# CogitoNTNU/geoguessr-ai

Hardware: AMD Instinct MI355X
Metric: images/sec TinyViT-21M-224 train, 4-heading batch (higher is better)
Workload: dtype fp32 (bf16x3 split MFMA); 1 GPU; tiny_vit_21m_224 4x224x224 panoramas, fwd+bwd+AdamW, soft-CE over 12647 geocells, freeze_all_but_last_stage, DropPath, train-mode BN; panoramas_per_gpu=256, images_per_gpu=1024, global_batch_panoramas=256, parallelism=dp1, precision=fp32_split

## Files before the change

### geoguessr-ai_amd/csrc/attention.hip

```cpp
#include "common.h"
#include <stdlib.h>
#include "../../include/gg.h"
int gg_attention_flash_bwd_impl(const GgAttnArgs* a, int dtype, int forward_rounded_bias, void* stream);

struct AttnParams {
    const bf16* qkv; int64_t ld;
    int q_off, k_off, v_off, head_stride;
    bf16* out; int64_t ldo;
    const bf16* bias; int nbias;
    int ws, nWx, nWy, H, W;
    int ws_inv;
    int N;
    int nh;
    float scale;
    const bf16* dout; int64_t lddo;
    bf16* dqkv;
    float* dbias;
    float* dbias_part;
    float* lse;
};

__device__ __forceinline__ int attn_origin(const AttnParams& p, int w) {
    if (p.ws == 0) return w * p.N;
    const int per_img = p.nWx * p.nWy;
// ... 614 lines not shown
    __shared__ __attribute__((aligned(16))) float row_lse[2][Np], row_delta[2][Np];
    __shared__ float dbias_s[DBIAS ? DBC * 256 : 1];
    __shared__ __attribute__((aligned(4))) unsigned char ci[Np], cj[Np];
    const int bid = gg_xcd_remap(blockIdx.x, gridDim.x);
    const int wb = bid / p.nh, h = bid % p.nh;
    const int lane = threadIdx.x & 63, wave = threadIdx.x >> 6;
    const int lr = lane & 15, lg = lane >> 4;
    const int qcol = p.q_off + h * p.head_stride, kcol = p.k_off + h * p.head_stride, vcol = p.v_off + h * p.head_stride;
    const int ocol = h * D;
    const int nt = (p.N + 15) / 16;
    const int ti = wave * 16 + lr;
    for (int t = threadIdx.x; t < Np; t += blockDim.x) {
        const int tt = min(t, p.N - 1), i = (tt * p.ws_inv) >> 16;
        ci[t] = p.ws ? (unsigned char)i : 0;
        cj[t] = p.ws ? (unsigned char)(tt - i * p.ws) : 0;
    }
    if (DBIAS) { for (int t = threadIdx.x; t < DBC * 256; t += blockDim.x) dbias_s[t] = 0.f; }
    u32x2 bq[NKT], bk[NKT];
#pragma unroll
    for (int kt = 0; kt < NKT; ++kt) {
        const int c0 = kt * 16 + lg * 4;
        bq[kt] = p.bias ? *reinterpret_cast<const u32x2*>(p.bias + ((int64_t)h * Np + ti) * Np + c0) : attn_mask_raw(c0, p.N);
        bk[kt] = p.bias ? *reinterpret_cast<const u32x2*>(p.bias + ((int64_t)h * Np + min(ti, p.N - 1)) * Np + c0) : attn_mask_raw(c0, p.N);
    }
    const float c2 = p.scale * 1.4426950408889634f;
    const int w0 = wb * GW, w1 = min(num_windows, w0 + GW);
    bf16x8 qr[IT], kr[IT], vr[IT], dr[IT], orr[IT];
    float lse_r = 0.f;
    auto fetch = [&](int w) {
        const int origin = attn_origin(p, w);
        int tokv[IT];
        attn_stage_tokens<D, Np>(p, origin, tokv);
        attn_load_rows<D, Np>(qr, p.qkv, p.ld, qcol, tokv);
        attn_load_rows<D, Np>(kr, p.qkv, p.ld, kcol, tokv);
        attn_load_rows<D, Np>(vr, p.qkv, p.ld, vcol, tokv);
        attn_load_rows<D, Np>(dr, p.dout, p.lddo, ocol, tokv);
        attn_load_rows<D, Np>(orr, p.out, p.ldo, ocol, tokv);
        if (threadIdx.x < Np) {
            const int tk = attn_token(p, origin, threadIdx.x);
            lse_r = tk >= 0 ? -1.4426950408889634f * p.lse[(int64_t)tk * p.nh + h] : 0.f;
        }
    };
    f32x4 dsum[DBIAS ? NKT : 1];
#pragma unroll
    for (int kt = 0; kt < (DBIAS ? NKT : 1); ++kt) dsum[kt] = (f32x4){0.f, 0.f, 0.f, 0.f};
    if (w0 < w1) fetch(w0);
    for (int w = w0; w < w1; ++w) {
        const int sel = (w - w0) & 1;
        bf16* Qs = img[sel][0]; bf16* Ks = img[sel][1]; bf16* Vs = img[sel][2]; bf16* dOs = img[sel][3];
        attn_store_rows<D, Np>(Qs, RS, qr);
        attn_store_rows<D, Np>(Ks, RS, kr);
        attn_store_rows<D, Np>(Vs, RS, vr);
        attn_store_rows<D, Np>(dOs, RS, dr);
        if (threadIdx.x < Np) row_lse[sel][threadIdx.x] = lse_r;
#pragma unroll
        for (int i = 0; i < IT; ++i) {
            const int idx = threadIdx.x + i * 256;
            float sm = 0.f;
#pragma unroll
            for (int j = 0; j < 8; ++j) sm += (float)dr[i][j] * (float)orr[i][j];
#pragma unroll
            for (int o = 1; o < CH; o <<= 1) sm += __shfl_xor(sm, o, 64);
            if (idx < Np * CH && (idx % CH) == 0) row_delta[sel][idx / CH] = -sm;
        }
        const int origin = attn_origin(p, w);
        const int tok_own = wave < nt ? attn_token(p, origin, ti) : -1;
        __syncthreads();
        if (w + 1 < w1) fetch(w + 1);
        if (wave < nt) {
            {
                bf16x8 qf[KS], dof[KS];
#pragma unroll
                for (int ks = 0; ks < KS; ++ks) {
                    qf[ks] = attn_lds_row_frag(Qs, RS, ti, ks * 32 + lg * 8);
                    dof[ks] = attn_lds_row_frag(dOs, RS, ti, ks * 32 + lg * 8);
                }
                const float nlse_q = row_lse[sel][ti], ndelta_q = row_delta[sel][ti];
                f32x4 dq[DT];
#pragma unroll
                for (int dt = 0; dt < DT; ++dt) dq[dt] = (f32x4){0.f, 0.f, 0.f, 0.f};
#pragma unroll
                for (int kp = 0; kp < NKT / 2; ++kp) {
                    f32x4 dst[2];
#pragma unroll
                    for (int u = 0; u < 2; ++u) {
                        const int kt = kp * 2 + u;
                        f32x4 acc = attn_bias_cvt(bq[kt]), acc2 = {ndelta_q, ndelta_q, ndelta_q, ndelta_q};
#pragma unroll
                        for (int ks = 0; ks < KS; ++ks) {
                            const bf16x8 kf = attn_lds_row_frag(Ks, RS, kt * 16 + lr, ks * 32 + lg * 8);
                            const bf16x8 vf = attn_lds_row_frag(Vs, RS, kt * 16 + lr, ks * 32 + lg * 8);
                            acc = __builtin_amdgcn_mfma_f32_16x16x32_bf16(kf, qf[ks], acc, 0, 0, 0);
                            acc2 = __builtin_amdgcn_mfma_f32_16x16x32_bf16(vf, dof[ks], acc2, 0, 0, 0);
                        }
                        const int key0 = kt * 16 + lg * 4;
#pragma unroll
                        for (int r = 0; r < 4; ++r) acc2[r] *= __builtin_amdgcn_exp2f(fmaf(acc[r], c2, nlse_q));
                        if (DBIAS) dsum[kt] += acc2;
                        dst[u] = acc2;
                    }
                    const bf16x8 df = attn_pack(dst[0], dst[1]);
#pragma unroll
                    for (int dt = 0; dt < DT; ++dt) {
                        const bf16x8 kf = attn_lds_tr_frag(Ks, RS, dt * 16, kp * 32, lr, lg);
                        dq[dt] = __builtin_amdgcn_mfma_f32_16x16x32_bf16(kf, df, dq[dt], 0, 0, 0);
                    }
                }
                if (tok_own >= 0) {
#pragma unroll
                    for (int dt = 0; dt < DT; ++dt) {
                        bf16x4 ov = {(bf16)(dq[dt][0] * p.scale), (bf16)(dq[dt][1] * p.scale), (bf16)(dq[dt][2] * p.scale), (bf16)(dq[dt][3] * p.scale)};
                        *reinterpret_cast<bf16x4*>(p.dqkv + (int64_t)tok_own * p.ld + qcol + dt * 16 + lg * 4) = ov;
                    }
                }
            }
            {
                bf16x8 kf[KS], vf[KS];
#pragma unroll
                for (int ks = 0; ks < KS; ++ks) {
                    kf[ks] = attn_lds_row_frag(Ks, RS, ti, ks * 32 + lg * 8);
                    vf[ks] = attn_lds_row_frag(Vs, RS, ti, ks * 32 + lg * 8);
                }
                f32x4 dk[DT], dv[DT];
#pragma unroll
                for (int dt = 0; dt < DT; ++dt) { dk[dt] = (f32x4){0.f, 0.f, 0.f, 0.f}; dv[dt] = (f32x4){0.f, 0.f, 0.f, 0.f}; }
#pragma unroll
                for (int qp = 0; qp < NKT / 2; ++qp) {
                    f32x4 pt[2], dst[2];
#pragma unroll
                    for (int u = 0; u < 2; ++u) {
                        const int qt = qp * 2 + u;
                        const int q0 = qt * 16 + lg * 4;
                        const f32x4 l4 = *reinterpret_cast<const f32x4*>(&row_lse[sel][q0]);
                        f32x4 acc = attn_bias_cvt(bk[qt]), acc2 = *reinterpret_cast<const f32x4*>(&row_delta[sel][q0]);
#pragma unroll
                        for (int ks = 0; ks < KS; ++ks) {
                            const bf16x8 qf = attn_lds_row_frag(Qs, RS, qt * 16 + lr, ks * 32 + lg * 8);
                            const bf16x8 dof = attn_lds_row_frag(dOs, RS, qt * 16 + lr, ks * 32 + lg * 8);
                            acc = __builtin_amdgcn_mfma_f32_16x16x32_bf16(qf, kf[ks], acc, 0, 0, 0);
                            acc2 = __builtin_amdgcn_mfma_f32_16x16x32_bf16(dof, vf[ks], acc2, 0, 0, 0);
                        }
#pragma unroll
                        for (int r = 0; r < 4; ++r) {
                            const float pr = __builtin_amdgcn_exp2f(fmaf(acc[r], c2, l4[r]));
                            acc[r] = pr;
                            acc2[r] *= pr;
                        }
                        pt[u] = acc;
                        dst[u] = acc2;
                    }
                    const bf16x8 pf = attn_pack(pt[0], pt[1]);
                    const bf16x8 df = attn_pack(dst[0], dst[1]);
#pragma unroll
                    for (int dt = 0; dt < DT; ++dt) {
                        const bf16x8 qtf = attn_lds_tr_frag(Qs, RS, dt * 16, qp * 32, lr, lg);
                        const bf16x8 dotf = attn_lds_tr_frag(dOs, RS, dt * 16, qp * 32, lr, lg);
                        dk[dt] = __builtin_amdgcn_mfma_f32_16x16x32_bf16(qtf, df, dk[dt], 0, 0, 0);
                        dv[dt] = __builtin_amdgcn_mfma_f32_16x16x32_bf16(dotf, pf, dv[dt], 0, 0, 0);
                    }
                }
                if (tok_own >= 0) {
#pragma unroll
                    for (int dt = 0; dt < DT; ++dt) {
                        bf16x4 a = {(bf16)(dk[dt][0] * p.scale), (bf16)(dk[dt][1] * p.scale), (bf16)(dk[dt][2] * p.scale), (bf16)(dk[dt][3] * p.scale)};
                        bf16x4 b = {(bf16)dv[dt][0], (bf16)dv[dt][1], (bf16)dv[dt][2], (bf16)dv[dt][3]};
                        *reinterpret_cast<bf16x4*>(p.dqkv + (int64_t)tok_own * p.ld + kcol + dt * 16 + lg * 4) = a;
                        *reinterpret_cast<bf16x4*>(p.dqkv + (int64_t)tok_own * p.ld + vcol + dt * 16 + lg * 4) = b;
                    }
                }
            }
        }
    }
    if (DBIAS) {
        if (wave < nt && ti < p.N) {
            const int qci = ci[ti], qcj = cj[ti];
#pragma unroll
            for (int kt = 0; kt < NKT; ++kt) {
                const int key0 = kt * 16 + lg * 4;
#pragma unroll
                for (int r = 0; r < 4; ++r)
                    if (key0 + r < p.N) atomicAdd(&dbias_s[(lr & (DBC - 1)) * 256 + abs(qci - (int)ci[key0 + r]) * p.ws + abs(qcj - (int)cj[key0 + r])], dsum[kt][r]);
            }
        }
        __syncthreads();
        for (int t = threadIdx.x; t < p.nbias; t += blockDim.x) {
            float sum = 0.f;
#pragma unroll
            for (int c = 0; c < DBC; ++c) sum += dbias_s[c * 256 + t];
            if (p.dbias_part) p.dbias_part[((int64_t)wb * p.nh + h) * p.nbias + t] = sum;
            else atomicAdd(&p.dbias[h * p.nbias + t], sum);
        }
    }
}

__global__ void attn_dbias_final_kernel(const float* __restrict__ rows, int nrows, int W, float* __restrict__ dbias) {
    const int i = blockIdx.x * blockDim.x + threadIdx.x;
    if (i >= W) return;
    double s = 0.0;
    for (int r = 0; r < nrows; ++r) s += (double)rows[(int64_t)r * W + i];
    dbias[i] += (float)s;
}

static int attn_fill(AttnParams& p, const GgAttnArgs* a, const char* who) {
    GG_CHECK(a && a->qkv, "%s: null qkv", who);
    GG_CHECK(a->head_dim == 32 || a->head_dim == 64, "%s: head_dim must be 32 or 64 (got %d)", who, a->head_dim);
    GG_CHECK(a->tokens_per_window > 0 && a->tokens_per_window <= 256,
             "%s: %d tokens per window unsupported (max 256: full-row softmax in registers)", who, a->tokens_per_window);
    GG_CHECK(a->num_windows > 0 && a->num_heads > 0, "%s: bad window/head count", who);
    GG_CHECK((a->ld & 7) == 0 && (a->q_off & 7) == 0 && (a->k_off & 7) == 0 && (a->v_off & 7) == 0 && (a->head_stride & 7) == 0,
             "%s: qkv offsets/strides must be multiples of 8 elements", who);
    if (a->window_size > 0) {
        GG_CHECK(a->window_size * a->window_size == a->tokens_per_window, "%s: window_size^2 != tokens_per_window", who);
        GG_CHECK(a->map_h % a->window_size == 0 && a->map_w % a->window_size == 0, "%s: map not divisible by window", who);
        GG_CHECK(a->num_windows % ((a->map_h / a->window_size) * (a->map_w / a->window_size)) == 0, "%s: window count", who);
        GG_CHECK(a->window_size <= 16, "%s: window_size > 16 unsupported", who);
    }
    if (a->bias || a->dbias) GG_CHECK(a->window_size > 0 && a->tokens_per_window <= 256, "%s: bias needs a window geometry", who);
    if (a->bias) GG_CHECK(((uintptr_t)a->bias & 7) == 0, "%s: expanded bias must be 8-byte aligned", who);
    p.qkv = (const bf16*)a->qkv; p.ld = a->ld;
    p.q_off = a->q_off; p.k_off = a->k_off; p.v_off = a->v_off; p.head_stride = a->head_stride;
    p.out = (bf16*)a->out; p.ldo = a->ldo;
    p.bias = (const bf16*)a->bias; p.nbias = a->window_size * a->window_size;
    p.ws = a->window_size;
    p.ws_inv = a->window_size ? (65536 + a->window_size - 1) / a->window_size : 0;
    p.H = a->map_h; p.W = a->map_w;
    p.nWx = a->window_size ? a->map_w / a->window_size : 1;
    p.nWy = a->window_size ? a->map_h / a->window_size : 1;
    p.N = a->tokens_per_window; p.nh = a->num_heads; p.scale = a->scale;
    p.dout = (const bf16*)a->dout; p.lddo = a->lddo; p.dqkv = (bf16*)a->dqkv; p.dbias = a->dbias; p.dbias_part = a->dbias ? a->dbias_scratch : nullptr; p.lse = a->lse;
    return 0;
}
static int attn_nkt(int N) { return N <= 64 ? 4 : (N <= 160 ? 10 : (N <= 224 ? 14 : 16)); }
extern "C" int gg_attention_padded_tokens(int tokens_per_window) { return 16 * attn_nkt(tokens_per_window); }
extern "C" int gg_attention_expand_bias(const float* table, int num_heads, int window_size, float scale, void* full, void* stream) {
    GG_CHECK(table && full && num_heads > 0 && window_size > 0 && window_size <= 16 && scale > 0.f, "gg_attention_expand_bias: bad args");
    const int N = window_size * window_size, Np = 16 * attn_nkt(N);
    const int64_t total = (int64_t)num_heads * Np * Np;
    hipLaunchKernelGGL(attn_expand_bias_kernel, dim3((unsigned)std::min<int64_t>(gg_cdiv(total, 256), 4096)), dim3(256), 0, (hipStream_t)stream,
                       table, num_heads, window_size, N, Np, 1.0f / scale, (bf16*)full);
    GG_LAUNCH_CHECK();
    return 0;
}

static bool attn_use_flash(const GgAttnArgs* a) { return a && (a->tokens_per_window > 256 || a->window_size > 16); }
static bool attn_use_split_bwd(const GgAttnArgs* a) {
    static const bool nosplit = gg_dev_env("GG_ATTN_NO_SPLIT") != nullptr;
    if (!a || nosplit || a->head_dim != 32 || a->window_size <= 0) return false;
    const int nt16 = (a->tokens_per_window + 15) / 16;
    return (nt16 == 13 || nt16 == 9) && (!a->bias || a->bias_table);
}
extern "C" int gg_attention_fwd(const GgAttnArgs* a, void* stream) {
    if (attn_use_flash(a)) {
        GG_CHECK(!a->bias || a->bias_table, "gg_attention_fwd: this window shape takes the bias as bias_table (compact f32)");
        return gg_attention_flash_fwd(a, 0, stream);
    }
    AttnParams p;
    GG_TRY(attn_fill(p, a, "gg_attention_fwd"));
    GG_CHECK(a->out && (a->ldo & 3) == 0, "gg_attention_fwd: bad out");
    dim3 grid((unsigned)(a->num_windows * a->num_heads)), block(256);
    hipStream_t s = (hipStream_t)stream;
    GG_PROF(GG_CAT_ATTN, 4.0 * a->num_windows * a->num_heads * (double)p.N * p.N * a->head_dim, 8.0 * a->num_windows * a->num_heads * (double)p.N * a->head_dim, stream);
    const int nkt = attn_nkt(p.N);
#define GG_FWD(D_, K_) hipLaunchKernelGGL((attn_fwd_kernel<D_, K_>), grid, block, 0, s, p)
    static const char* small_env = gg_dev_env("GG_ATTN_SMALL");
    if (a->head_dim == 32 && nkt == 4 && !(small_env && small_env[0] == '0') && a->num_windows >= 64) {
        constexpr int GW = 8;
        const dim3 g2((unsigned)(gg_cdiv(a->num_windows, GW) * a->num_heads));
        hipLaunchKernelGGL((attn_fwd_small_kernel<32, GW>), g2, block, 0, s, p, a->num_windows);
        GG_LAUNCH_CHECK();
        return 0;
    }
    if (a->head_dim == 32) {
        if (nkt == 4) GG_FWD(32, 4); else if (nkt == 10) GG_FWD(32, 10); else if (nkt == 14) GG_FWD(32, 14); else GG_FWD(32, 16);
    } else {
        if (nkt == 4) GG_FWD(64, 4); else if (nkt == 10) GG_FWD(64, 10); else if (nkt == 14) GG_FWD(64, 14); else GG_FWD(64, 16);
    }
#undef GG_FWD
    GG_LAUNCH_CHECK();
    return 0;
}
extern "C" int gg_attention_fwd_f16(const GgAttnArgs* a, void* stream) {
    GG_CHECK(a && !a->bias && !a->bias_table, "gg_attention_fwd_f16: the fp16 forward takes no bias");
    if (attn_use_flash(a)) return gg_attention_flash_fwd(a, 2, stream);
    AttnParams p;
    GG_TRY(attn_fill(p, a, "gg_attention_fwd_f16"));
    GG_CHECK(a->out && (a->ldo & 3) == 0, "gg_attention_fwd_f16: bad out");
    dim3 grid((unsigned)(a->num_windows * a->num_heads)), block(256);
    hipStream_t s = (hipStream_t)stream;
    GG_PROF(GG_CAT_ATTN, 4.0 * a->num_windows * a->num_heads * (double)p.N * p.N * a->head_dim, 8.0 * a->num_windows * a->num_heads * (double)p.N * a->head_dim, stream);
    const int nkt = attn_nkt(p.N);
#define GG_FWD16(D_, K_) hipLaunchKernelGGL((attn_fwd_kernel<D_, K_, f16>), grid, block, 0, s, p)
    if (a->head_dim == 32) {
        if (nkt == 4) GG_FWD16(32, 4); else if (nkt == 10) GG_FWD16(32, 10); else if (nkt == 14) GG_FWD16(32, 14); else GG_FWD16(32, 16);
    } else {
        if (nkt == 4) GG_FWD16(64, 4); else if (nkt == 10) GG_FWD16(64, 10); else if (nkt == 14) GG_FWD16(64, 14); else GG_FWD16(64, 16);
    }
#undef GG_FWD16
    GG_LAUNCH_CHECK();
    return 0;
}
extern "C" int gg_attention_bwd(const GgAttnArgs* a, void* stream) {
    if (attn_use_flash(a) || attn_use_split_bwd(a)) {
        GG_CHECK(!a->bias || a->bias_table, "gg_attention_bwd: this window shape takes the bias as bias_table (compact f32)");
        return gg_attention_flash_bwd_impl(a, 0, 1, stream);
    }
    AttnParams p;
    GG_TRY(attn_fill(p, a, "gg_attention_bwd"));
    GG_CHECK(a->dout && a->dqkv && (a->lddo & 7) == 0, "gg_attention_bwd: bad dout/dqkv");
    GG_CHECK(a->lse && a->out && (a->ldo & 7) == 0, "gg_attention_bwd: needs the forward's lse and out");
    GG_CHECK(a->head_dim == 32, "gg_attention_bwd: only head_dim 32 (TinyViT) is built");
    dim3 grid((unsigned)(a->num_windows * a->num_heads)), block(256);
    hipStream_t s = (hipStream_t)stream;
    GG_PROF(GG_CAT_ATTN, 10.0 * a->num_windows * a->num_heads * (double)p.N * p.N * a->head_dim, 16.0 * a->num_windows * a->num_heads * (double)p.N * a->head_dim, stream);
    const int nkt = attn_nkt(p.N);
#define GG_BWD(K_)                                                                                       \
    do {                                                                                                 \
        if (p.dbias) hipLaunchKernelGGL((attn_bwd_kernel<32, K_, true>), grid, block, 0, s, p);          \
        else hipLaunchKernelGGL((attn_bwd_kernel<32, K_, false>), grid, block, 0, s, p);                 \
    } while (0)
    static const char* small_env = gg_dev_env("GG_ATTN_SMALL");
    int part_rows = a->num_windows;
    if (nkt == 4 && !(small_env && small_env[0] == '0') && a->num_windows >= 64) {
        constexpr int GW = 8;
        part_rows = (int)gg_cdiv(a->num_windows, GW);
        const dim3 g2((unsigned)(part_rows * a->num_heads));
        if (p.dbias) hipLaunchKernelGGL((attn_bwd_small_kernel<32, GW, true>), g2, block, 0, s, p, a->num_windows);
        else hipLaunchKernelGGL((attn_bwd_small_kernel<32, GW, false>), g2, block, 0, s, p, a->num_windows);
    } else if (nkt == 4) GG_BWD(4); else if (nkt == 10) GG_BWD(10); else if (nkt == 14) GG_BWD(14); else GG_BWD(16);
#undef GG_BWD
    if (p.dbias && p.dbias_part) {
        const int Wd = p.nh * p.nbias;
        const float* rows; int nrows;
        gg_reduce_rows(p.dbias_part, part_rows, Wd, s, &rows, &nrows);
        hipLaunchKernelGGL(attn_dbias_final_kernel, dim3((unsigned)gg_cdiv(Wd, 256)), dim3(256), 0, s, rows, nrows, Wd, p.dbias);
    }
    GG_LAUNCH_CHECK();
    return 0;
}
```

### geoguessr-ai_amd/csrc/attention_split.h

```cpp
typedef short sp_s4 __attribute__((ext_vector_type(4)));

template <int NPL> struct Sp8T { bf16x8 p[NPL]; };
template <int NPL> struct Sp4T { sp_s4 p[NPL]; };

struct Sp1 { bf16 a, b, c; };
__device__ __forceinline__ Sp1 sp_split1(float x) {
    Sp1 o;
    o.a = (bf16)x;
    const float r1 = x - (float)o.a;
    o.b = (bf16)r1;
    o.c = (bf16)(r1 - (float)o.b);
    return o;
}
template <int NPL> __device__ __forceinline__ Sp8T<NPL> sp_split8(const f32x4& lo, const f32x4& hi) {
    Sp8T<NPL> o;
    if constexpr (NPL == 1) {
#pragma unroll
        for (int j = 0; j < 4; ++j) { o.p[0][j] = (bf16)lo[j]; o.p[0][4 + j] = (bf16)hi[j]; }
    } else {
#pragma unroll
        for (int j = 0; j < 4; ++j) {
            const Sp1 u = sp_split1(lo[j]), v = sp_split1(hi[j]);
            o.p[0][j] = u.a; o.p[1][j] = u.b; o.p[2][j] = u.c;
            o.p[0][4 + j] = v.a; o.p[1][4 + j] = v.b; o.p[2][4 + j] = v.c;
        }
    }
    return o;
}
template <int NPL> __device__ __forceinline__ f32x4 sp_mma32(const Sp8T<NPL>& a, const Sp8T<NPL>& b, f32x4 acc) {
    if constexpr (NPL == 1) return __builtin_amdgcn_mfma_f32_16x16x32_bf16(a.p[0], b.p[0], acc, 0, 0, 0);
    else {
        acc = __builtin_amdgcn_mfma_f32_16x16x32_bf16(a.p[0], b.p[2], acc, 0, 0, 0);
        acc = __builtin_amdgcn_mfma_f32_16x16x32_bf16(a.p[1], b.p[1], acc, 0, 0, 0);
        acc = __builtin_amdgcn_mfma_f32_16x16x32_bf16(a.p[2], b.p[0], acc, 0, 0, 0);
        acc = __builtin_amdgcn_mfma_f32_16x16x32_bf16(a.p[0], b.p[1], acc, 0, 0, 0);
        acc = __builtin_amdgcn_mfma_f32_16x16x32_bf16(a.p[1], b.p[0], acc, 0, 0, 0);
        acc = __builtin_amdgcn_mfma_f32_16x16x32_bf16(a.p[0], b.p[0], acc, 0, 0, 0);
        return acc;
    }
}
template <typename T> struct SpLd8;
template <> struct SpLd8<float> {
    static __device__ __forceinline__ void load(__amdgpu_buffer_rsrc_t rs, int off, f32x4& lo, f32x4& hi) {
        lo = Bld<float>::load(rs, off); hi = Bld<float>::load(rs, off == FL_OOB ? FL_OOB : off + 16);
    }
};
template <> struct SpLd8<bf16> {
    static __device__ __forceinline__ void load(__amdgpu_buffer_rsrc_t rs, int off, f32x4& lo, f32x4& hi) {
        const bf16x8 v = __builtin_bit_cast(bf16x8, __builtin_amdgcn_raw_buffer_load_b128(rs, off, 0, 0));
#pragma unroll
        for (int j = 0; j < 4; ++j) { lo[j] = (float)v[j]; hi[j] = (float)v[4 + j]; }
    }
};
__device__ __forceinline__ int sp_off(int row, int ch) { return row * 32 + ((ch ^ ((-(row >> 2)) & 3)) << 3); }
template <typename T, int NPL>
__device__ __forceinline__ void sp_stage(const FlashParams& p, __amdgpu_buffer_rsrc_t rs, int ldb, int colb, bf16* X, int R) {
    const int PL = R * 32;
    for (int id = threadIdx.x; id < R * 4; id += blockDim.x) {
        const int row = id >> 2, ch = id & 3;
        const int off = row < p.N ? fl_tokrel(p, row) * ldb + colb + ch * 8 * (int)sizeof(T) : FL_OOB;
        f32x4 lo, hi;
        SpLd8<T>::load(rs, off, lo, hi);
        const Sp8T<NPL> s = sp_split8<NPL>(lo, hi);
        const int o = sp_off(row, ch);
#pragma unroll
        for (int pl = 0; pl < NPL; ++pl) *reinterpret_cast<bf16x8*>(X + pl * PL + o) = s.p[pl];
    }
}
template <int NPL> __device__ __forceinline__ Sp8T<NPL> sp_frag(const bf16* X, int PL, int row, int lg) {
    Sp8T<NPL> f;
    const int o = sp_off(row, lg);
#pragma unroll
    for (int pl = 0; pl < NPL; ++pl) f.p[pl] = *reinterpret_cast<const bf16x8*>(X + pl * PL + o);
    return f;
}
template <int NPL> __device__ __forceinline__ Sp4T<NPL> sp_frag_t(const bf16* X, int PL, int row0, int c, int lr, int lg) {
    const int row = row0 + 4 * lg + (lr >> 2), col = 16 * c + 4 * (lr & 3);
    const int o = sp_off(row, col >> 3) + (col & 7);
    Sp4T<NPL> f;
#pragma unroll
    for (int pl = 0; pl < NPL; ++pl) f.p[pl] = __builtin_amdgcn_ds_read_tr16_b64_v4i16((__attribute__((address_space(3))) sp_s4*)(X + pl * PL + o));
    return f;
}
template <int NPL> __device__ __forceinline__ Sp8T<NPL> sp_frag_t2(const bf16* X, int PL, int row0, int row1, int c, int lr, int lg) {
    const Sp4T<NPL> a = sp_frag_t<NPL>(X, PL, row0, c, lr, lg), b = sp_frag_t<NPL>(X, PL, row1, c, lr, lg);
    Sp8T<NPL> f;
#pragma unroll
    for (int pl = 0; pl < NPL; ++pl) {
        union { sp_s4 s[2]; bf16x8 v; } u;
        u.s[0] = a.p[pl]; u.s[1] = b.p[pl];
        f.p[pl] = u.v;
    }
    return f;
}

template <typename T, int NPL, int NT>
__global__ __launch_bounds__(64 * NT) void flash_fwd_split_kernel(FlashParams p) {
    constexpr int D = 32, R = 16 * NT, PL = R * 32, ES = (int)sizeof(T);
    typedef Sp8T<NPL> Sp8;
    extern __shared__ __attribute__((aligned(16))) float fsm[];
    bf16* Kp = reinterpret_cast<bf16*>(fsm);
    bf16* Vp = Kp + NPL * PL;
    float* btab = reinterpret_cast<float*>(Vp + NPL * PL);
    int* klin = reinterpret_cast<int*>(btab + p.nbpad);
    const int h = blockIdx.x % p.nh, w = blockIdx.x / p.nh;
    const int lane = threadIdx.x & 63, wave = __builtin_amdgcn_readfirstlane(threadIdx.x >> 6);
    const int lr = lane & 15, lg = lane >> 4;
    const int64_t origin = fl_origin(p, w);
    const int hc = h * p.head_stride;
    const bool has_bias = p.bias_table != nullptr;
    const int span = fl_span(p);
    const int ldb = (int)p.ld * ES, ldob = (int)p.ldo * ES;
    const __amdgpu_buffer_rsrc_t rsQKV = fl_rsrc(reinterpret_cast<const T*>(p.qkv) + origin * p.ld, span * ldb);
    const __amdgpu_buffer_rsrc_t rsOUT = fl_rsrc(reinterpret_cast<T*>(p.out) + origin * p.ldo, span * ldob);
    const __amdgpu_buffer_rsrc_t rsLSE = fl_rsrc(p.lse ? p.lse + origin * p.nh : nullptr, p.lse ? span * p.nh * 4 : 0);
    const int srow = threadIdx.x >> 2, sch = threadIdx.x & 3;
    const int soff = srow < p.N ? fl_tokrel(p, srow) * ldb + (hc + sch * 8) * ES : FL_OOB;
    f32x4 klo, khi, vlo, vhi, qlo, qhi;
    SpLd8<T>::load(rsQKV, soff == FL_OOB ? FL_OOB : soff + p.k_off * ES, klo, khi);
    SpLd8<T>::load(rsQKV, soff == FL_OOB ? FL_OOB : soff + p.v_off * ES, vlo, vhi);
    const int strip = wave;
    const int qi = strip * 16 + lr;
    const bool qok = qi < p.N;
    const int qrel = qok ? fl_tokrel(p, qi) : 0;
    SpLd8<T>::load(rsQKV, qok ? qrel * ldb + (p.q_off + hc + 8 * lg) * ES : FL_OOB, qlo, qhi);
    if (has_bias) fl_stage_bias(p, h, btab);
    if (has_bias) fl_stage_coords(p, 0, klin, R);
    {
        const Sp8 k3 = sp_split8<NPL>(klo, khi), v3 = sp_split8<NPL>(vlo, vhi);
        const int o = sp_off(srow, sch);
#pragma unroll
        for (int pl = 0; pl < NPL; ++pl) {
            *reinterpret_cast<bf16x8*>(Kp + pl * PL + o) = k3.p[pl];
            *reinterpret_cast<bf16x8*>(Vp + pl * PL + o) = v3.p[pl];
        }
    }
    const Sp8 q3 = sp_split8<NPL>(qlo, qhi);
    const int qlin = has_bias ? fl_lin4(p, min(qi, p.N - 1)) + 4 * (p.ws - 1) * 2 * p.ws : 0;
    const float sc2 = p.scale * 1.4426950408889634f;
    __syncthreads();
    if (strip * 16 >= p.N) return;
    f32x4 st[NT];
    float mx = -INFINITY;
#pragma unroll
    for (int kt = 0; kt < NT; ++kt) {
        f32x4 s = {0.f, 0.f, 0.f, 0.f};
        if (16 * kt + 15 >= p.N) {
#pragma unroll
            for (int r = 0; r < 4; ++r) s[r] = (16 * kt + 4 * lg + r < p.N) ? 0.f : -INFINITY;
        }
        s = sp_mma32<NPL>(sp_frag<NPL>(Kp, PL, 16 * kt + lr, lg), q3, s);
        f32x4 bia = {0.f, 0.f, 0.f, 0.f};
        if (has_bias) {
            const i32x4 kl4 = *reinterpret_cast<const i32x4*>(klin + 16 * kt + 4 * lg);
#pragma unroll
            for (int r = 0; r < 4; ++r) bia[r] = *reinterpret_cast<const float*>(reinterpret_cast<const char*>(btab) + (qlin - kl4[r]));
        }
#pragma unroll
        for (int r = 0; r < 4; ++r) { s[r] = fmaf(s[r], sc2, bia[r]); mx = fmaxf(mx, s[r]); }
        st[kt] = s;
    }
    mx = fmaxf(mx, __shfl_xor(mx, 16, 64));
    mx = fmaxf(mx, __shfl_xor(mx, 32, 64));
    float l = 0.f;
    f32x4 oacc[2] = {{0.f, 0.f, 0.f, 0.f}, {0.f, 0.f, 0.f, 0.f}};
#pragma unroll
    for (int kt = 0; kt < NT; kt += 2) {
        f32x4 e0, e1 = {0.f, 0.f, 0.f, 0.f};
#pragma unroll
        for (int r = 0; r < 4; ++r) { e0[r] = __builtin_amdgcn_exp2f(st[kt][r] - mx); l += e0[r]; }
        if (kt + 1 < NT) {
#pragma unroll
            for (int r = 0; r < 4; ++r) { e1[r] = __builtin_amdgcn_exp2f(st[kt + 1 < NT ? kt + 1 : kt][r] - mx); l += e1[r]; }
        }
        const Sp8 p3 = sp_split8<NPL>(e0, e1);
#pragma unroll
        for (int c = 0; c < 2; ++c) oacc[c] = sp_mma32<NPL>(sp_frag_t2<NPL>(Vp, PL, 16 * kt, kt + 1 < NT ? 16 * (kt + 1) : 16 * kt, c, lr, lg), p3, oacc[c]);
    }
    l += __shfl_xor(l, 16, 64);
    l += __shfl_xor(l, 32, 64);
    const float inv = 1.0f / l;
#pragma unroll
    for (int c = 0; c < 2; ++c) Bld<T>::store(rsOUT, qok ? qrel * ldob + (h * D + 16 * c + 4 * lg) * ES : FL_OOB, oacc[c] * inv);
    if (p.lse) __builtin_amdgcn_raw_buffer_store_b32(__builtin_bit_cast(unsigned, mx * 0.6931471805599453f + __logf(l)), rsLSE,
                                                     (qok && lg == 0) ? (qrel * p.nh + h) * 4 : FL_OOB, 0, 0);
}
size_t sp_lds_fwd(const FlashParams& p, int npl) { return (size_t)2 * npl * p.npad * 32 * 2 + ((size_t)p.nbpad + p.npad) * 4; }

template <typename T, int NPL, bool DBIAS, int NT>
__global__ __launch_bounds__(64 * ((NT + 1) / 2)) void flash_bwd_split_kernel(FlashParams p) {
    constexpr int D = 32, NP = (NT + 1) / 2, R = 32 * NP, PL = R * 32, RS = D + 4, TS = 20, ES = (int)sizeof(T);
    typedef Sp8T<NPL> Sp8;
    extern __shared__ __attribute__((aligned(16))) float fsm[];
    bf16* Qp = reinterpret_cast<bf16*>(fsm);
    bf16* Op = Qp + NPL * PL;
    float* dQs = reinterpret_cast<float*>(Op + NPL * PL);
    float* btab = dQs + R * RS;
    float* dbt = btab + p.nbpad;
    float* lse_s = dbt + (DBIAS ? p.nbpad : 0);
    float* del_s = lse_s + R;
    int* qlin = reinterpret_cast<int*>(del_s + R);
    float* Gt = reinterpret_cast<float*>(qlin + R);
    const int wh = blockIdx.x;
    const int h = wh % p.nh, w = wh / p.nh;
    const int lane = threadIdx.x & 63, wave = __builtin_amdgcn_readfirstlane(threadIdx.x >> 6);
    const int lr = lane & 15, lg = lane >> 4;
    const int64_t origin = fl_origin(p, w);
    const int hc = h * p.head_stride;
    const bool has_bias = p.bias_table != nullptr;
    const int nb = p.ws * p.ws;
    const int w2 = 2 * p.ws - 1;
    const int span = fl_span(p);
    const int ldb = (int)p.ld * ES, lddob = (int)p.lddo * ES, ldob = (int)p.ldo * ES;
    const __amdgpu_buffer_rsrc_t rsQKV = fl_rsrc(reinterpret_cast<const T*>(p.qkv) + origin * p.ld, span * ldb);
    const __amdgpu_buffer_rsrc_t rsDO = fl_rsrc(reinterpret_cast<const T*>(p.dout) + origin * p.lddo, span * lddob);
    const __amdgpu_buffer_rsrc_t rsO = fl_rsrc(reinterpret_cast<const T*>(p.out) + origin * p.ldo, span * ldob);
    const __amdgpu_buffer_rsrc_t rsLSE = fl_rsrc(p.lse + origin * p.nh, span * p.nh * 4);
    const __amdgpu_buffer_rsrc_t rsDQKV = fl_rsrc(reinterpret_cast<T*>(p.dqkv) + origin * p.ld, span * ldb);
    f32x4 qv[2][2], gv[2][2], ov[2][2];
    float lsev[2];
#pragma unroll
    for (int i = 0; i < 2; ++i) {
        const int id = threadIdx.x + i * (64 * NP), row = id >> 2, ch = id & 3;
        const bool ok = row < p.N;
        const int rel = ok ? fl_tokrel(p, row) : 0;
        const int oq = ok ? rel * ldb + (p.q_off + hc + ch * 8) * ES : FL_OOB, og = ok ? rel * lddob + (h * D + ch * 8) * ES : FL_OOB, oo = ok ? rel * ldob + (h * D + ch * 8) * ES : FL_OOB;
        SpLd8<T>::load(rsQKV, oq, qv[i][0], qv[i][1]);
        SpLd8<T>::load(rsDO, og, gv[i][0], gv[i][1]);
        SpLd8<T>::load(rsO, oo, ov[i][0], ov[i][1]);
        lsev[i] = __builtin_bit_cast(float, __builtin_amdgcn_raw_buffer_load_b32(rsLSE, (ok && ch == 0) ? (rel * p.nh + h) * 4 : FL_OOB, 0, 0));
    }
    Sp8 k3[2], v3[2], kT3[2];
    int klin[2], krow[2];
    bool kok[2];
    f32x4 kv[2][2], vv[2][2];
#pragma unroll
    for (int s = 0; s < 2; ++s) {
        const int ki = 32 * wave + 16 * s + lr;
        kok[s] = ki < p.N;
        krow[s] = kok[s] ? fl_tokrel(p, ki) * ldb : FL_OOB;
        SpLd8<T>::load(rsQKV, kok[s] ? krow[s] + (p.k_off + hc + 8 * lg) * ES : FL_OOB, kv[s][0], kv[s][1]);
        SpLd8<T>::load(rsQKV, kok[s] ? krow[s] + (p.v_off + hc + 8 * lg) * ES : FL_OOB, vv[s][0], vv[s][1]);
        klin[s] = has_bias ? fl_lin4(p, min(ki, p.N - 1)) - 4 * (p.ws - 1) * 2 * p.ws : 0;
    }
    if (has_bias) {
        fl_stage_bias(p, h, btab);
        if (NPL == 1 && p.round_bias) {
            __syncthreads();
            for (int i = threadIdx.x; i < w2 * w2; i += blockDim.x) {
                const float b = btab[i] * 0.6931471805599453f;
                btab[i] = (float)(bf16)(b * -p.neg_inv_scale) * (p.scale * 1.4426950408889634f);
            }
        }
    } else if (threadIdx.x < 4) btab[threadIdx.x] = 0.f;
    if (DBIAS) for (int i = threadIdx.x; i < w2 * w2; i += blockDim.x) dbt[i] = 0.f;
    for (int i = threadIdx.x; i < R * RS / 4; i += blockDim.x) reinterpret_cast<f32x4*>(dQs)[i] = (f32x4){0.f, 0.f, 0.f, 0.f};
    if (has_bias) fl_stage_coords(p, 0, qlin, R); else for (int i = threadIdx.x; i < R; i += blockDim.x) qlin[i] = 0;
    const float sc2 = p.scale * 1.4426950408889634f;
    float* slot = Gt + wave * (16 * TS);
    float* tslot = reinterpret_cast<float*>(Qp) + wave * (2 * 16 * TS);
    {
        f32x4 kt[2][2];
#pragma unroll
        for (int s = 0; s < 2; ++s) {
            k3[s] = sp_split8<NPL>(kv[s][0], kv[s][1]);
            v3[s] = sp_split8<NPL>(vv[s][0], vv[s][1]);
            *reinterpret_cast<f32x4*>(tslot + (lg >> 1) * (16 * TS) + lr * TS + 8 * (lg & 1)) = kv[s][0];
            *reinterpret_cast<f32x4*>(tslot + (lg >> 1) * (16 * TS) + lr * TS + 8 * (lg & 1) + 4) = kv[s][1];
#pragma unroll
            for (int c = 0; c < 2; ++c)
#pragma unroll
                for (int r = 0; r < 4; ++r) kt[c][s][r] = tslot[c * (16 * TS) + (4 * lg + r) * TS + lr];
        }
#pragma unroll
        for (int c = 0; c < 2; ++c) kT3[c] = sp_split8<NPL>(kt[c][0], kt[c][1]);
    }
    f32x4 dk[2][2], dv[2][2];
#pragma unroll
    for (int s = 0; s < 2; ++s)
#pragma unroll
        for (int c = 0; c < 2; ++c) dk[s][c] = dv[s][c] = (f32x4){0.f, 0.f, 0.f, 0.f};
    __syncthreads();
#pragma unroll
    for (int i = 0; i < 2; ++i) {
        const int id = threadIdx.x + i * (64 * NP), row = id >> 2, ch = id & 3;
        const Sp8 q3 = sp_split8<NPL>(qv[i][0], qv[i][1]), g3 = sp_split8<NPL>(gv[i][0], gv[i][1]);
        const int o = sp_off(row, ch);
#pragma unroll
        for (int pl = 0; pl < NPL; ++pl) {
            *reinterpret_cast<bf16x8*>(Qp + pl * PL + o) = q3.p[pl];
            *reinterpret_cast<bf16x8*>(Op + pl * PL + o) = g3.p[pl];
        }
        float dsum = 0.f;
#pragma unroll
        for (int j = 0; j < 4; ++j) dsum = fmaf(gv[i][0][j], ov[i][0][j], dsum);
#pragma unroll
        for (int j = 0; j < 4; ++j) dsum = fmaf(gv[i][1][j], ov[i][1][j], dsum);
        dsum += __shfl_xor(dsum, 1, 64);
        dsum += __shfl_xor(dsum, 2, 64);
        if (ch == 0) {
            del_s[row] = -dsum;
            lse_s[row] = row < p.N ? -1.4426950408889634f * lsev[i] : -INFINITY;
        }
    }
    __syncthreads();

    int pair = wave;
    for (int t = 0; t < NP; ++t) {
        f32x4 pr[2][2], ds[2][2];
#pragma unroll
        for (int a = 0; a < 2; ++a) {
            const int tile = 2 * pair + a, q4 = tile * 16 + 4 * lg;
            const Sp8 qf = sp_frag<NPL>(Qp, PL, tile * 16 + lr, lg), of = sp_frag<NPL>(Op, PL, tile * 16 + lr, lg);
            const f32x4 st0 = {0.f, 0.f, 0.f, 0.f}, nl4 = *reinterpret_cast<const f32x4*>(lse_s + q4), dp0 = *reinterpret_cast<const f32x4*>(del_s + q4);
            const i32x4 ql4 = *reinterpret_cast<const i32x4*>(qlin + q4);
            f32x4 dT[2];
#pragma unroll
            for (int s = 0; s < 2; ++s) {
                const f32x4 st = sp_mma32<NPL>(qf, k3[s], st0), dp = sp_mma32<NPL>(of, v3[s], dp0);
                const i32x4 boff4 = ql4 - klin[s];
                f32x4 bia;
#pragma unroll
                for (int r = 0; r < 4; ++r) bia[r] = *reinterpret_cast<const float*>(reinterpret_cast<const char*>(btab) + boff4[r]);
#pragma unroll
                for (int r = 0; r < 4; ++r) {
                    const float e = __builtin_amdgcn_exp2f(fmaf(st[r], sc2, bia[r] + nl4[r]));
                    const float g = e * dp[r];
                    pr[a][s][r] = e;
                    ds[a][s][r] = g;
                    slot[(4 * lg + r) * TS + lr] = g;
                    if (DBIAS && kok[s] && q4 + r < p.N) atomicAdd(reinterpret_cast<float*>(reinterpret_cast<char*>(dbt) + boff4[r]), g);
                }
                dT[s] = *reinterpret_cast<const f32x4*>(slot + lr * TS + 4 * lg);
            }
            const f32x4 d0 = dT[0], d1 = dT[1];
            const Sp8 dst = sp_split8<NPL>(d0, d1);
            float* dQt = dQs + (tile * 16 + lr) * RS + 4 * lg;
#pragma unroll
            for (int c = 0; c < 2; ++c) {
                const f32x4 dq = sp_mma32<NPL>(kT3[c], dst, *reinterpret_cast<const f32x4*>(dQt + 16 * c));
                *reinterpret_cast<f32x4*>(dQt + 16 * c) = dq;
            }
        }
        Sp8 ot[2], qt[2];
#pragma unroll
        for (int c = 0; c < 2; ++c) {
            ot[c] = sp_frag_t2<NPL>(Op, PL, 32 * pair, 32 * pair + 16, c, lr, lg);
            qt[c] = sp_frag_t2<NPL>(Qp, PL, 32 * pair, 32 * pair + 16, c, lr, lg);
        }
#pragma unroll
        for (int s = 0; s < 2; ++s) {
            const Sp8 p3 = sp_split8<NPL>(pr[0][s], pr[1][s]), g3 = sp_split8<NPL>(ds[0][s], ds[1][s]);
#pragma unroll
            for (int c = 0; c < 2; ++c) {
                dv[s][c] = sp_mma32<NPL>(ot[c], p3, dv[s][c]);
                dk[s][c] = sp_mma32<NPL>(qt[c], g3, dk[s][c]);
            }
        }
        __syncthreads();
        pair = pair + 1 == NP ? 0 : pair + 1;
    }
#pragma unroll
    for (int s = 0; s < 2; ++s)
#pragma unroll
        for (int c = 0; c < 2; ++c) {
            Bld<T>::store(rsDQKV, kok[s] ? krow[s] + (p.k_off + hc + 16 * c + 4 * lg) * ES : FL_OOB, dk[s][c] * p.scale);
            Bld<T>::store(rsDQKV, kok[s] ? krow[s] + (p.v_off + hc + 16 * c + 4 * lg) * ES : FL_OOB, dv[s][c]);
        }
    constexpr int CH = D / 4;
    for (int id = threadIdx.x; id < p.N * CH; id += blockDim.x) {
        const int row = id / CH, ch = id % CH;
        const f32x4 v = *reinterpret_cast<const f32x4*>(dQs + row * RS + ch * 4);
        Bld<T>::store(rsDQKV, fl_tokrel(p, row) * ldb + (p.q_off + hc + ch * 4) * ES, v * p.scale);
    }
    if (DBIAS) {
        for (int i = threadIdx.x; i < nb; i += blockDim.x) {
            const int ady = fl_div(i, p.rcp_ws), adx = i - ady * p.ws, c0 = (p.ws - 1) * w2 + (p.ws - 1);
            float tt = dbt[c0 + ady * w2 + adx];
            if (ady) tt += dbt[c0 - ady * w2 + adx];
            if (adx) tt += dbt[c0 + ady * w2 - adx];
            if (ady && adx) tt += dbt[c0 - ady * w2 - adx];
            if (p.dbias_part) p.dbias_part[((int64_t)w * p.nh + h) * nb + i] = tt;
            else atomicAdd(&p.dbias[h * nb + i], tt);
        }
    }
}
size_t sp_lds_bwd(const FlashParams& p, bool dbias, int npl) {
    const size_t np = (p.npad / 16 + 1) / 2, R = 32 * np;
    return 2 * npl * R * 64 + (R * 36 + (size_t)p.nbpad * (dbias ? 2 : 1) + 3 * R + np * 320) * 4;
}
```

Measured before the change: 5633 images/s.

## Split dS before LDS transpose, swizzle dQ accumulator, packed bf16 splitting in split attention

Measured after the change: 5668 images/s (median of 6 runs). Within noise of the previous version (+0.6%).

```diff
diff --git a/geoguessr-ai_amd/csrc/attention.hip b/geoguessr-ai_amd/csrc/attention.hip
--- a/geoguessr-ai_amd/csrc/attention.hip
+++ b/geoguessr-ai_amd/csrc/attention.hip
@@ -940,7 +940,7 @@
 extern "C" int gg_attention_bwd(const GgAttnArgs* a, void* stream) {
     if (attn_use_flash(a) || attn_use_split_bwd(a)) {
         GG_CHECK(!a->bias || a->bias_table, "gg_attention_bwd: this window shape takes the bias as bias_table (compact f32)");
-        return gg_attention_flash_bwd_impl(a, 0, 1, stream);
+        return gg_attention_flash_bwd_impl(a, 0, attn_use_flash(a) ? 0 : 1, stream);
     }
     AttnParams p;
     GG_TRY(attn_fill(p, a, "gg_attention_bwd"));
diff --git a/geoguessr-ai_amd/csrc/attention_split.h b/geoguessr-ai_amd/csrc/attention_split.h
--- a/geoguessr-ai_amd/csrc/attention_split.h
+++ b/geoguessr-ai_amd/csrc/attention_split.h
@@ -3,30 +3,61 @@
 template <int NPL> struct Sp8T { bf16x8 p[NPL]; };
 template <int NPL> struct Sp4T { sp_s4 p[NPL]; };
 
-struct Sp1 { bf16 a, b, c; };
-__device__ __forceinline__ Sp1 sp_split1(float x) {
-    Sp1 o;
-    o.a = (bf16)x;
-    const float r1 = x - (float)o.a;
-    o.b = (bf16)r1;
-    o.c = (bf16)(r1 - (float)o.b);
+typedef bf16 sp_bf2 __attribute__((ext_vector_type(2)));
+typedef float sp_f2 __attribute__((ext_vector_type(2)));
+template <int NPL> __device__ __forceinline__ void sp_split2(float x0, float x1, unsigned (&w)[NPL]) {
+#pragma unroll
+    for (int pl = 0; pl < NPL; ++pl) {
+        w[pl] = __builtin_bit_cast(unsigned, __builtin_convertvector((sp_f2){x0, x1}, sp_bf2));
+        if (pl + 1 < NPL) {
+            x0 -= __builtin_bit_cast(float, w[pl] << 16);
+            x1 -= __builtin_bit_cast(float, w[pl] & 0xffff0000u);
+        }
+    }
+}
+template <int NPL> __device__ __forceinline__ Sp8T<NPL> sp_split8(const f32x4& lo, const f32x4& hi) {
+    typedef unsigned u32x4 __attribute__((ext_vector_type(4)));
+    u32x4 v[NPL];
+#pragma unroll
+    for (int j = 0; j < 4; ++j) {
+        unsigned w[NPL];
+        sp_split2<NPL>(j < 2 ? lo[2 * j] : hi[2 * j - 4], j < 2 ? lo[2 * j + 1] : hi[2 * j - 3], w);
+#pragma unroll
+        for (int pl = 0; pl < NPL; ++pl) v[pl][j] = w[pl];
+    }
+    Sp8T<NPL> o;
+#pragma unroll
+    for (int pl = 0; pl < NPL; ++pl) o.p[pl] = __builtin_bit_cast(bf16x8, v[pl]);
     return o;
 }
-template <int NPL> __device__ __forceinline__ Sp8T<NPL> sp_split8(const f32x4& lo, const f32x4& hi) {
-    Sp8T<NPL> o;
-    if constexpr (NPL == 1) {
-#pragma unroll
-        for (int j = 0; j < 4; ++j) { o.p[0][j] = (bf16)lo[j]; o.p[0][4 + j] = (bf16)hi[j]; }
-    } else {
-#pragma unroll
-        for (int j = 0; j < 4; ++j) {
-            const Sp1 u = sp_split1(lo[j]), v = sp_split1(hi[j]);
-            o.p[0][j] = u.a; o.p[1][j] = u.b; o.p[2][j] = u.c;
-            o.p[0][4 + j] = v.a; o.p[1][4 + j] = v.b; o.p[2][4 + j] = v.c;
-        }
-    }
+template <int NPL> __device__ __forceinline__ Sp4T<NPL> sp_split4(const f32x4& x) {
+    typedef unsigned u32x2 __attribute__((ext_vector_type(2)));
+    u32x2 v[NPL];
+#pragma unroll
+    for (int j = 0; j < 2; ++j) {
+        unsigned w[NPL];
+        sp_split2<NPL>(x[2 * j], x[2 * j + 1], w);
+#pragma unroll
+        for (int pl = 0; pl < NPL; ++pl) v[pl][j] = w[pl];
+    }
+    Sp4T<NPL> o;
+#pragma unroll
+    for (int pl = 0; pl < NPL; ++pl) o.p[pl] = __builtin_bit_cast(sp_s4, v[pl]);
     return o;
 }
+template <int NPL> __device__ __forceinline__ Sp8T<NPL> sp_cat(const Sp4T<NPL>& a, const Sp4T<NPL>& b) {
+    Sp8T<NPL> f;
+#pragma unroll
+    for (int pl = 0; pl < NPL; ++pl) {
+        union { sp_s4 s[2]; bf16x8 v; } u;
+        u.s[0] = a.p[pl]; u.s[1] = b.p[pl];
+        f.p[pl] = u.v;
+    }
+    return f;
+}
+typedef __attribute__((address_space(3))) float sp_lds_f32;
+__device__ __forceinline__ int sp_lds_addr(const void* ptr) { return (int)(uintptr_t)(__attribute__((address_space(3))) const void*)ptr; }
+__device__ __forceinline__ float sp_lds_ld(int addr) { return *(const sp_lds_f32*)(uintptr_t)(unsigned)addr; }
 template <int NPL> __device__ __forceinline__ f32x4 sp_mma32(const Sp8T<NPL>& a, const Sp8T<NPL>& b, f32x4 acc) {
     if constexpr (NPL == 1) return __builtin_amdgcn_mfma_f32_16x16x32_bf16(a.p[0], b.p[0], acc, 0, 0, 0);
     else {
@@ -83,15 +114,7 @@
     return f;
 }
 template <int NPL> __device__ __forceinline__ Sp8T<NPL> sp_frag_t2(const bf16* X, int PL, int row0, int row1, int c, int lr, int lg) {
-    const Sp4T<NPL> a = sp_frag_t<NPL>(X, PL, row0, c, lr, lg), b = sp_frag_t<NPL>(X, PL, row1, c, lr, lg);
-    Sp8T<NPL> f;
-#pragma unroll
-    for (int pl = 0; pl < NPL; ++pl) {
-        union { sp_s4 s[2]; bf16x8 v; } u;
-        u.s[0] = a.p[pl]; u.s[1] = b.p[pl];
-        f.p[pl] = u.v;
-    }
-    return f;
+    return sp_cat<NPL>(sp_frag_t<NPL>(X, PL, row0, c, lr, lg), sp_frag_t<NPL>(X, PL, row1, c, lr, lg));
 }
 
 template <typename T, int NPL, int NT>
@@ -124,8 +147,13 @@
     const bool qok = qi < p.N;
     const int qrel = qok ? fl_tokrel(p, qi) : 0;
     SpLd8<T>::load(rsQKV, qok ? qrel * ldb + (p.q_off + hc + 8 * lg) * ES : FL_OOB, qlo, qhi);
-    if (has_bias) fl_stage_bias(p, h, btab);
-    if (has_bias) fl_stage_coords(p, 0, klin, R);
+    if (has_bias) {
+        fl_stage_bias(p, h, btab);
+        fl_stage_coords(p, 0, klin, R);
+    } else {
+        if (threadIdx.x < 4) btab[threadIdx.x] = 0.f;
+        if (threadIdx.x < R) klin[threadIdx.x] = 0;
+    }
     {
         const Sp8 k3 = sp_split8<NPL>(klo, khi), v3 = sp_split8<NPL>(vlo, vhi);
         const int o = sp_off(srow, sch);
@@ -136,26 +164,23 @@
         }
     }
     const Sp8 q3 = sp_split8<NPL>(qlo, qhi);
-    const int qlin = has_bias ? fl_lin4(p, min(qi, p.N - 1)) + 4 * (p.ws - 1) * 2 * p.ws : 0;
+    const int qb = sp_lds_addr(btab) + (has_bias ? fl_lin4(p, min(qi, p.N - 1)) + 4 * (p.ws - 1) * 2 * p.ws : 0);
     const float sc2 = p.scale * 1.4426950408889634f;
     __syncthreads();
     if (strip * 16 >= p.N) return;
     f32x4 st[NT];
     float mx = -INFINITY;
+    f32x4 slast;
+#pragma unroll
+    for (int r = 0; r < 4; ++r) slast[r] = (16 * (NT - 1) + 4 * lg + r < p.N) ? 0.f : -INFINITY;
 #pragma unroll
     for (int kt = 0; kt < NT; ++kt) {
-        f32x4 s = {0.f, 0.f, 0.f, 0.f};
-        if (16 * kt + 15 >= p.N) {
-#pragma unroll
-            for (int r = 0; r < 4; ++r) s[r] = (16 * kt + 4 * lg + r < p.N) ? 0.f : -INFINITY;
-        }
+        f32x4 s = kt == NT - 1 ? slast : (f32x4){0.f, 0.f, 0.f, 0.f};
         s = sp_mma32<NPL>(sp_frag<NPL>(Kp, PL, 16 * kt + lr, lg), q3, s);
-        f32x4 bia = {0.f, 0.f, 0.f, 0.f};
-        if (has_bias) {
-            const i32x4 kl4 = *reinterpret_cast<const i32x4*>(klin + 16 * kt + 4 * lg);
-#pragma unroll
-            for (int r = 0; r < 4; ++r) bia[r] = *reinterpret_cast<const float*>(reinterpret_cast<const char*>(btab) + (qlin - kl4[r]));
-        }
+        const i32x4 kl4 = *reinterpret_cast<const i32x4*>(klin + 16 * kt + 4 * lg);
+        f32x4 bia;
+#pragma unroll
+        for (int r = 0; r < 4; ++r) bia[r] = sp_lds_ld(qb - kl4[r]);
 #pragma unroll
         for (int r = 0; r < 4; ++r) { s[r] = fmaf(s[r], sc2, bia[r]); mx = fmaxf(mx, s[r]); }
         st[kt] = s;
@@ -189,18 +214,19 @@
 
 template <typename T, int NPL, bool DBIAS, int NT>
 __global__ __launch_bounds__(64 * ((NT + 1) / 2)) void flash_bwd_split_kernel(FlashParams p) {
-    constexpr int D = 32, NP = (NT + 1) / 2, R = 32 * NP, PL = R * 32, RS = D + 4, TS = 20, ES = (int)sizeof(T);
+    constexpr int D = 32, NP = (NT + 1) / 2, R = 32 * NP, PL = R * 32, TS = 20, ES = (int)sizeof(T);
     typedef Sp8T<NPL> Sp8;
+    typedef Sp4T<NPL> Sp4;
     extern __shared__ __attribute__((aligned(16))) float fsm[];
     bf16* Qp = reinterpret_cast<bf16*>(fsm);
     bf16* Op = Qp + NPL * PL;
     float* dQs = reinterpret_cast<float*>(Op + NPL * PL);
-    float* btab = dQs + R * RS;
+    float* btab = dQs + R * D;
     float* dbt = btab + p.nbpad;
     float* lse_s = dbt + (DBIAS ? p.nbpad : 0);
     float* del_s = lse_s + R;
     int* qlin = reinterpret_cast<int*>(del_s + R);
-    float* Gt = reinterpret_cast<float*>(qlin + R);
+    bf16* Gt = reinterpret_cast<bf16*>(qlin + R);
     const int wh = blockIdx.x;
     const int h = wh % p.nh, w = wh / p.nh;
     const int lane = threadIdx.x & 63, wave = __builtin_amdgcn_readfirstlane(threadIdx.x >> 6);
@@ -242,6 +268,7 @@
         SpLd8<T>::load(rsQKV, kok[s] ? krow[s] + (p.k_off + hc + 8 * lg) * ES : FL_OOB, kv[s][0], kv[s][1]);
         SpLd8<T>::load(rsQKV, kok[s] ? krow[s] + (p.v_off + hc + 8 * lg) * ES : FL_OOB, vv[s][0], vv[s][1]);
         klin[s] = has_bias ? fl_lin4(p, min(ki, p.N - 1)) - 4 * (p.ws - 1) * 2 * p.ws : 0;
+        klin[s] -= sp_lds_addr(btab);
     }
     if (has_bias) {
         fl_stage_bias(p, h, btab);
@@ -254,10 +281,10 @@
         }
     } else if (threadIdx.x < 4) btab[threadIdx.x] = 0.f;
     if (DBIAS) for (int i = threadIdx.x; i < w2 * w2; i += blockDim.x) dbt[i] = 0.f;
-    for (int i = threadIdx.x; i < R * RS / 4; i += blockDim.x) reinterpret_cast<f32x4*>(dQs)[i] = (f32x4){0.f, 0.f, 0.f, 0.f};
+    for (int i = threadIdx.x; i < R * D / 4; i += blockDim.x) reinterpret_cast<f32x4*>(dQs)[i] = (f32x4){0.f, 0.f, 0.f, 0.f};
     if (has_bias) fl_stage_coords(p, 0, qlin, R); else for (int i = threadIdx.x; i < R; i += blockDim.x) qlin[i] = 0;
     const float sc2 = p.scale * 1.4426950408889634f;
-    float* slot = Gt + wave * (16 * TS);
+    bf16* slot = Gt + wave * (NPL * 256);
     float* tslot = reinterpret_cast<float*>(Qp) + wave * (2 * 16 * TS);
     {
         f32x4 kt[2][2];
@@ -307,39 +334,43 @@
 
     int pair = wave;
     for (int t = 0; t < NP; ++t) {
-        f32x4 pr[2][2], ds[2][2];
+        f32x4 pr[2][2];
+        Sp4 gs[2][2];
 #pragma unroll
         for (int a = 0; a < 2; ++a) {
             const int tile = 2 * pair + a, q4 = tile * 16 + 4 * lg;
             const Sp8 qf = sp_frag<NPL>(Qp, PL, tile * 16 + lr, lg), of = sp_frag<NPL>(Op, PL, tile * 16 + lr, lg);
             const f32x4 st0 = {0.f, 0.f, 0.f, 0.f}, nl4 = *reinterpret_cast<const f32x4*>(lse_s + q4), dp0 = *reinterpret_cast<const f32x4*>(del_s + q4);
             const i32x4 ql4 = *reinterpret_cast<const i32x4*>(qlin + q4);
-            f32x4 dT[2];
+            Sp4 dth[2];
 #pragma unroll
             for (int s = 0; s < 2; ++s) {
                 const f32x4 st = sp_mma32<NPL>(qf, k3[s], st0), dp = sp_mma32<NPL>(of, v3[s], dp0);
-                const i32x4 boff4 = ql4 - klin[s];
-                f32x4 bia;
-#pragma unroll
-                for (int r = 0; r < 4; ++r) bia[r] = *reinterpret_cast<const float*>(reinterpret_cast<const char*>(btab) + boff4[r]);
+                const i32x4 baddr4 = ql4 - klin[s];
+                f32x4 bia, g;
+#pragma unroll
+                for (int r = 0; r < 4; ++r) bia[r] = sp_lds_ld(baddr4[r]);
 #pragma unroll
                 for (int r = 0; r < 4; ++r) {
                     const float e = __builtin_amdgcn_exp2f(fmaf(st[r], sc2, bia[r] + nl4[r]));
-                    const float g = e * dp[r];
                     pr[a][s][r] = e;
-                    ds[a][s][r] = g;
-                    slot[(4 * lg + r) * TS + lr] = g;
-                    if (DBIAS && kok[s] && q4 + r < p.N) atomicAdd(reinterpret_cast<float*>(reinterpret_cast<char*>(dbt) + boff4[r]), g);
+                    g[r] = e * dp[r];
+                    if (DBIAS && kok[s] && q4 + r < p.N) atomicAdd(reinterpret_cast<float*>(reinterpret_cast<char*>(dbt) + (baddr4[r] - sp_lds_addr(btab))), g[r]);
                 }
-                dT[s] = *reinterpret_cast<const f32x4*>(slot + lr * TS + 4 * lg);
+                gs[a][s] = sp_split4<NPL>(g);
+#pragma unroll
+                for (int pl = 0; pl < NPL; ++pl)
+                    *reinterpret_cast<sp_s4*>(slot + pl * 256 + lr * 16 + ((lg ^ ((lr >> 2) & 3)) << 2)) = gs[a][s].p[pl];
+#pragma unroll
+                for (int pl = 0; pl < NPL; ++pl)
+                    dth[s].p[pl] = __builtin_amdgcn_ds_read_tr16_b64_v4i16((__attribute__((address_space(3))) sp_s4*)(slot + pl * 256 + (4 * lg + (lr >> 2)) * 16 + (((lr & 3) ^ lg) << 2)));
             }
-            const f32x4 d0 = dT[0], d1 = dT[1];
-            const Sp8 dst = sp_split8<NPL>(d0, d1);
-            float* dQt = dQs + (tile * 16 + lr) * RS + 4 * lg;
+            const Sp8 dst = sp_cat<NPL>(dth[0], dth[1]);
+            float* dQt = dQs + (tile * 16 + lr) * D;
 #pragma unroll
             for (int c = 0; c < 2; ++c) {
-                const f32x4 dq = sp_mma32<NPL>(kT3[c], dst, *reinterpret_cast<const f32x4*>(dQt + 16 * c));
-                *reinterpret_cast<f32x4*>(dQt + 16 * c) = dq;
+                f32x4* dqp = reinterpret_cast<f32x4*>(dQt + (((lg + 4 * c) ^ (lr & 7)) << 2));
+                *dqp = sp_mma32<NPL>(kT3[c], dst, *dqp);
             }
         }
         Sp8 ot[2], qt[2];
@@ -350,7 +381,7 @@
         }
 #pragma unroll
         for (int s = 0; s < 2; ++s) {
-            const Sp8 p3 = sp_split8<NPL>(pr[0][s], pr[1][s]), g3 = sp_split8<NPL>(ds[0][s], ds[1][s]);
+            const Sp8 p3 = sp_split8<NPL>(pr[0][s], pr[1][s]), g3 = sp_cat<NPL>(gs[0][s], gs[1][s]);
 #pragma unroll
             for (int c = 0; c < 2; ++c) {
                 dv[s][c] = sp_mma32<NPL>(ot[c], p3, dv[s][c]);
@@ -370,7 +401,7 @@
     constexpr int CH = D / 4;
     for (int id = threadIdx.x; id < p.N * CH; id += blockDim.x) {
         const int row = id / CH, ch = id % CH;
-        const f32x4 v = *reinterpret_cast<const f32x4*>(dQs + row * RS + ch * 4);
+        const f32x4 v = *reinterpret_cast<const f32x4*>(dQs + row * D + ((ch ^ (row & 7)) << 2));
         Bld<T>::store(rsDQKV, fl_tokrel(p, row) * ldb + (p.q_off + hc + ch * 4) * ES, v * p.scale);
     }
     if (DBIAS) {
@@ -387,5 +418,5 @@
 }
 size_t sp_lds_bwd(const FlashParams& p, bool dbias, int npl) {
     const size_t np = (p.npad / 16 + 1) / 2, R = 32 * np;
-    return 2 * npl * R * 64 + (R * 36 + (size_t)p.nbpad * (dbias ? 2 : 1) + 3 * R + np * 320) * 4;
-}
+    return 2 * npl * R * 64 + (R * 32 + (size_t)p.nbpad * (dbias ? 2 : 1) + 3 * R) * 4 + np * npl * 512;
+}
```
